# facebookresearch/metamorph

Hardware: AMD Instinct MI355X
Metric: train tokens/sec (LLaMA-3-8B + SigLIP-SO400M, seq2048, 256 img toks), whole job (higher is better)
Workload: dtype bf16

## Files before the change

### metamorph_amd/csrc/gemm_bf16.hip

```cpp
#include "gemm_common.h"
#include "splitk.h"
#include <type_traits>
#include <cstdlib>

namespace {

MM_DEV void gemm_epilogue_swiglu(f32x4 (&acc)[8][4], const GemmArgs& a, unsigned char* smem, int m0, int tn, int wm, int wn, int wave, int lane) {
    constexpr int TN = 64;
    const int fr = lane & 15, fq = lane >> 4;
    const int M = a.M, I = (int)a.res_mod;
    float* stg = (float*)smem + wave * (16 * TN);
    const int row_l = lane >> 2, k4 = lane & 3;
    uint16_t* gu = (uint16_t*)a.C;
    uint16_t* act = (uint16_t*)a.res;
    const int ch0 = tn * 128 + wn * 32;
#pragma unroll
    for (int i = 0; i < 8; ++i) {
        __builtin_amdgcn_fence(__ATOMIC_RELEASE, "wavefront");
        __builtin_amdgcn_wave_barrier();
#pragma unroll
        for (int j = 0; j < 4; ++j)
#pragma unroll
            for (int r = 0; r < 4; ++r) stg[(fq * 4 + r) * TN + j * 16 + fr] = acc[i][j][r];
        __builtin_amdgcn_fence(__ATOMIC_RELEASE, "wavefront");
        __builtin_amdgcn_wave_barrier();
        const int grow = m0 + wm * 128 + i * 16 + row_l;
        if (grow < M) {
            float g[8], u[8], o[8];
            const f32x4 g0 = *(const f32x4*)(stg + row_l * TN + k4 * 8), g1 = *(const f32x4*)(stg + row_l * TN + k4 * 8 + 4);
            const f32x4 u0 = *(const f32x4*)(stg + row_l * TN + 32 + k4 * 8), u1 = *(const f32x4*)(stg + row_l * TN + 32 + k4 * 8 + 4);
            g[0] = g0.x; g[1] = g0.y; g[2] = g0.z; g[3] = g0.w; g[4] = g1.x; g[5] = g1.y; g[6] = g1.z; g[7] = g1.w;
            u[0] = u0.x; u[1] = u0.y; u[2] = u0.z; u[3] = u0.w; u[4] = u1.x; u[5] = u1.y; u[6] = u1.z; u[7] = u1.w;
            const u32x4 gp = pack8(g), up = pack8(u);
            const int ch = ch0 + k4 * 8;
            *(u32x4*)(gu + (int64_t)grow * a.ldc + ch) = gp;
            *(u32x4*)(gu + (int64_t)grow * a.ldc + I + ch) = up;
            float gb[8], ub[8];
            unpack8(gp, gb);
            unpack8(up, ub);
#pragma unroll
            for (int e = 0; e < 8; ++e) o[e] = round_bf(gb[e] / (1.0f + __expf(-gb[e]))) * ub[e];
            *(u32x4*)(act + (int64_t)grow * a.ldr + ch) = pack8(o);
        }
    }
}

constexpr int SWB_TROW = 144;
constexpr int SWB_T = 3 * 32 * SWB_TROW;
constexpr int SWB_LDS = 32768 + 8 * SWB_T;
MM_DEV void gemm_epilogue_swiglu_bwd(f32x4 (&acc)[8][4], const GemmArgs& a, unsigned char* smem, int m0, int n0, int wm, int wn, int wave, int lane) {
    constexpr int TN = 64, PF = 4;
    typedef __attribute__((ext_vector_type(4))) short s16x4;
    typedef __attribute__((address_space(3))) s16x4* lds4_t;
    const int fr = lane & 15, fq = lane >> 4;
    const int M = a.M, I = a.N;
    float* stg = (float*)smem + wave * (16 * TN);
    unsigned char* tile = smem + 32768 + wave * SWB_T;
    const int row_l = lane >> 2, k4 = lane & 3;
    const uint16_t* gu = a.res;
    uint16_t* dgu = (uint16_t*)a.C;
    const int c_wave = n0 + wn * 64;
    if (c_wave >= I) return;
    const int row0 = m0 + wm * 128 + row_l;
    u32x4 gq[PF][2], uq[PF][2];
    auto fetch = [&](int i, int slot) {
        const int grow = row0 + i * 16;
#pragma unroll
        for (int j8 = 0; j8 < 2; ++j8) {
            const int64_t ro = (int64_t)min(grow, M - 1) * a.ldr + c_wave + k4 * 16 + j8 * 8;
            gq[slot][j8] = *(const u32x4*)(gu + ro);
            uq[slot][j8] = *(const u32x4*)(gu + ro + I);
        }
    };
#pragma unroll
    for (int i = 0; i < PF; ++i) fetch(i, i);
#pragma unroll
    for (int ib = 0; ib < 4; ++ib) {
#pragma unroll
        for (int half = 0; half < 2; ++half) {
            const int i = ib * 2 + half;
            __builtin_amdgcn_fence(__ATOMIC_RELEASE, "wavefront");
            __builtin_amdgcn_wave_barrier();
#pragma unroll
            for (int j = 0; j < 4; ++j)
#pragma unroll
                for (int r = 0; r < 4; ++r) stg[(fq * 4 + r) * TN + j * 16 + fr] = acc[i][j][r];
            __builtin_amdgcn_fence(__ATOMIC_RELEASE, "wavefront");
            __builtin_amdgcn_wave_barrier();
            const int grow = row0 + i * 16;
            const bool live = grow < M;
#pragma unroll
            for (int j8 = 0; j8 < 2; ++j8) {
                const int c = k4 * 16 + j8 * 8;
                float daf[8], g[8], u[8], dg[8], du[8], av[8], da[8];
                const f32x4 s0 = *(const f32x4*)(stg + row_l * TN + c), s1 = *(const f32x4*)(stg + row_l * TN + c + 4);
                daf[0] = s0.x; daf[1] = s0.y; daf[2] = s0.z; daf[3] = s0.w; daf[4] = s1.x; daf[5] = s1.y; daf[6] = s1.z; daf[7] = s1.w;
                unpack8(pack8(daf), da);
                unpack8(gq[i % PF][j8], g);
                unpack8(uq[i % PF][j8], u);
#pragma unroll
                for (int e = 0; e < 8; ++e) {
                    const float sg = 1.0f / (1.0f + __expf(-g[e]));
                    const float silu = g[e] * sg;
                    av[e] = round_bf(silu) * u[e];
                    du[e] = da[e] * round_bf(silu);
                    dg[e] = da[e] * u[e] * (sg * (1.0f + g[e] * (1.0f - sg)));
                }
                const u32x4 pg = pack8(dg), pu = pack8(du), pa = pack8(av);
                if (live) {
                    const int64_t wo = (int64_t)grow * a.ldc + c_wave + c;
                    *(u32x4*)(dgu + wo) = pg;
                    *(u32x4*)(dgu + wo + I) = pu;
                }
                unsigned char* tp = tile + (half * 16 + row_l) * SWB_TROW + c * 2;
                *(u32x4*)(tp) = pa;
                *(u32x4*)(tp + 32 * SWB_TROW) = pg;
                *(u32x4*)(tp + 64 * SWB_TROW) = pu;
            }
            if (i + PF < 8) fetch(i + PF, i % PF);
        }
        __builtin_amdgcn_fence(__ATOMIC_RELEASE, "wavefront");
        __builtin_amdgcn_wave_barrier();
        const int r_base = m0 + wm * 128 + ib * 32;
        const int s_l = fr >> 2, j_l = fr & 3;
        const unsigned char* tb = tile + (8 * (fr & 3) + (fr >> 2)) * SWB_TROW + fq * 8;
#pragma unroll
        for (int q = 0; q < 3; ++q) {
#pragma unroll
            for (int it = 0; it < 4; ++it) {
                const s16x4 lo = __builtin_amdgcn_ds_read_tr16_b64_v4i16((lds4_t)(tb + q * 32 * SWB_TROW + it * 32));
                const s16x4 hi = __builtin_amdgcn_ds_read_tr16_b64_v4i16((lds4_t)(tb + (q * 32 + 4) * SWB_TROW + it * 32));
                const int ch = c_wave + it * 16 + fq * 4 + j_l;
                const int r8 = r_base + 8 * s_l;
                if (r8 < M) {
                    typedef __attribute__((ext_vector_type(8))) short s16x8;
                    uint16_t* outp = (q == 0 ? a.aux0 : a.aux1) + (int64_t)(q == 2 ? I + ch : ch) * a.ld_aux;
                    *(s16x8*)(outp + r8) = s16x8{lo[0], lo[1], lo[2], lo[3], hi[0], hi[1], hi[2], hi[3]};
                }
            }
        }
    }
}

MM_DEV void gemm_epilogue_rope(f32x4 (&acc)[8][4], const GemmArgs& a, unsigned char* smem, int m0, int n0, int wm, int wn, int wave, int lane) {
    constexpr int TN = 64;
    const int fr = lane & 15, fq = lane >> 4;
    const int M = a.M, L = (int)a.ld_aux, n_rot = (int)a.res_mod;
    float* stg = (float*)smem + wave * (16 * TN);
    const int row_l = lane >> 2, k4 = lane & 3;
    uint16_t* out = (uint16_t*)a.C;
    const int32_t* pos_off = (const int32_t*)a.bias;
    const int d1 = (wn & 1) * 32 + k4 * 8;
    const int col1 = n0 + (wn >> 1) * 128 + d1;
    const bool rot = col1 < n_rot;
#pragma unroll
    for (int i = 0; i < 8; ++i) {
        __builtin_amdgcn_fence(__ATOMIC_RELEASE, "wavefront");
        __builtin_amdgcn_wave_barrier();
#pragma unroll
        for (int j = 0; j < 4; ++j)
#pragma unroll
            for (int r = 0; r < 4; ++r) stg[(fq * 4 + r) * TN + j * 16 + fr] = acc[i][j][r];
        __builtin_amdgcn_fence(__ATOMIC_RELEASE, "wavefront");
        __builtin_amdgcn_wave_barrier();
        const int grow = m0 + wm * 128 + i * 16 + row_l;
        if (grow < M) {
            float a1[8], a2[8], x1[8], x2[8];
            const f32x4 p0 = *(const f32x4*)(stg + row_l * TN + k4 * 8), p1 = *(const f32x4*)(stg + row_l * TN + k4 * 8 + 4);
            const f32x4 q0 = *(const f32x4*)(stg + row_l * TN + 32 + k4 * 8), q1 = *(const f32x4*)(stg + row_l * TN + 32 + k4 * 8 + 4);
            a1[0] = p0.x; a1[1] = p0.y; a1[2] = p0.z; a1[3] = p0.w; a1[4] = p1.x; a1[5] = p1.y; a1[6] = p1.z; a1[7] = p1.w;
            a2[0] = q0.x; a2[1] = q0.y; a2[2] = q0.z; a2[3] = q0.w; a2[4] = q1.x; a2[5] = q1.y; a2[6] = q1.z; a2[7] = q1.w;
            u32x4 w1 = pack8(a1), w2 = pack8(a2);
            if (rot) {
                unpack8(w1, x1);
                unpack8(w2, x2);
                const int b = grow / L;
                const int l = grow - b * L + (pos_off ? pos_off[b] : 0);
                float c[8], sn[8], y1[8], y2[8];
                unpack8(*(const u32x4*)(a.aux0 + (int64_t)l * 128 + d1), c);
                unpack8(*(const u32x4*)(a.aux1 + (int64_t)l * 128 + d1), sn);
#pragma unroll
                for (int e = 0; e < 8; ++e) {
                    y1[e] = round_bf(x1[e] * c[e]) + round_bf(-x2[e] * sn[e]);
                    y2[e] = round_bf(x2[e] * c[e]) + round_bf(x1[e] * sn[e]);
                }
                w1 = pack8(y1); w2 = pack8(y2);
            }
            *(u32x4*)(out + (int64_t)grow * a.ldc + col1) = w1;
            *(u32x4*)(out + (int64_t)grow * a.ldc + col1 + 64) = w2;
        }
    }
}

template <int BM, int BN, int WM, int WN, bool GLDS, int PIPE = 0>
__global__ __launch_bounds__(WM* WN * 64) void gemm_nt_kernel(GemmArgs a) {
    constexpr int NT = WM * WN * 64, NW = WM * WN;
    constexpr int TM = BM / WM, TN = BN / WN, FM = TM / 16, FN = TN / 16;
    constexpr int A_BYTES = BM * 128, B_BYTES = BN * 128, STAGE = A_BYTES + B_BYTES;
    constexpr int AV = BM * 8 / NT, BV = BN * 8 / NT;
    constexpr int AI = BM / 8 / NW, BI = BN / 8 / NW;
    constexpr int GM = 8;
    static_assert(FM >= 1 && FN >= 2 && (FN % 2) == 0, "tile shape");
    static_assert(AV >= 1 && BV >= 1 && AI >= 1 && BI >= 1, "thread/tile ratio");

    extern __shared__ __attribute__((aligned(16))) unsigned char smem[];

    const int total = a.ntm * a.ntn;
    const int bid = blockIdx.x;
    const int q8 = total >> 3, r8 = total & 7;
    const int xcd = bid & 7, idx = bid >> 3;
    const int logical = (xcd < r8 ? xcd * (q8 + 1) : r8 * (q8 + 1) + (xcd - r8) * q8) + idx;
    const int gsize = GM * a.ntn;
    const int grp = logical / gsize;
    const int first_m = grp * GM;
    const int gm = min(a.ntm - first_m, GM);
    const int in_g = logical - grp * gsize;
    const int tm = first_m + in_g % gm;
    const int tn = in_g / gm;
    const int m0 = tm * BM, n0 = tn * BN;

    const int tid = threadIdx.x, lane = tid & 63, wave = tid >> 6;
    const int wm = wave / WN, wn = wave % WN;
    const int fr = lane & 15, fq = lane >> 4;
    const int sl = a.kslice ? (int)blockIdx.y : 0;
    const uint16_t* Ab = a.A + (int64_t)sl * a.kslice;
    const uint16_t* Bb = a.B + (int64_t)sl * a.kslice;
    const int M = a.M, N = a.N, K = a.kslice ? min(a.kslice, a.K - sl * a.kslice) : a.K;
    const int nk = (K + 63) >> 6;

    f32x4 acc[FM][FN];
#pragma unroll
    for (int i = 0; i < FM; ++i)
#pragma unroll
        for (int j = 0; j < FN; ++j) acc[i][j] = f32x4{0.f, 0.f, 0.f, 0.f};

    const int sw0 = ((fq) ^ (fr & 7)) << 4;
    const int sw1 = ((4 + fq) ^ (fr & 7)) << 4;
    const int a_off = (wm * TM + fr) * 128;
    const int b_off = A_BYTES + (wn * TN + fr) * 128;

    u32x4 ra[AV], rb[BV];

    auto gload = [&](int kt) {
        const int k0 = kt << 6;
#pragma unroll
        for (int i = 0; i < AV; ++i) {
            const int v = tid + i * NT, row = v >> 3, c = v & 7;
            const int gr = min(m0 + row, M - 1), k = k0 + c * 8;
            ra[i] = (k < K) ? *(const u32x4*)(Ab + (int64_t)gr * a.lda + k) : u32x4{0u, 0u, 0u, 0u};
        }
#pragma unroll
        for (int i = 0; i < BV; ++i) {
            const int v = tid + i * NT, row = v >> 3, c = v & 7;
            const int gr = min(n0 + row, N - 1), k = k0 + c * 8;
            rb[i] = (k < K) ? *(const u32x4*)(Bb + (int64_t)gr * a.ldb + k) : u32x4{0u, 0u, 0u, 0u};
        }
    };
    auto lstore = [&](int buf) {
        unsigned char* sb = smem + buf * STAGE;
#pragma unroll
        for (int i = 0; i < AV; ++i) {
            const int v = tid + i * NT, row = v >> 3, c = v & 7;
            *(u32x4*)(sb + row * 128 + ((c ^ (row & 7)) << 4)) = ra[i];
        }
#pragma unroll
        for (int i = 0; i < BV; ++i) {
            const int v = tid + i * NT, row = v >> 3, c = v & 7;
            *(u32x4*)(sb + A_BYTES + row * 128 + ((c ^ (row & 7)) << 4)) = rb[i];
        }
    };
    const int wave_s = __builtin_amdgcn_readfirstlane(wave);
    const uint16_t* srcA[AI];
    const uint16_t* srcB[BI];
    {
        const int rin = lane >> 3;
        const int c = (lane & 7) ^ rin;
#pragma unroll
        for (int i = 0; i < AI; ++i)
            srcA[i] = Ab + (int64_t)min(m0 + (i * NW + wave_s) * 8 + rin, M - 1) * a.lda + c * 8;
#pragma unroll
        for (int i = 0; i < BI; ++i)
            srcB[i] = Bb + (int64_t)min(n0 + (i * NW + wave_s) * 8 + rin, N - 1) * a.ldb + c * 8;
    }
    auto gdma = [&](int kt, int buf) {
        const int64_t k0 = kt << 6;
        unsigned char* sb = smem + buf * STAGE + wave_s * 1024;
#pragma unroll
        for (int i = 0; i < AI; ++i)
            __builtin_amdgcn_global_load_lds((gptr_t)(srcA[i] + k0), (lptr_t)(sb + i * NW * 1024), 16, 0, 0);
#pragma unroll
        for (int i = 0; i < BI; ++i)
            __builtin_amdgcn_global_load_lds((gptr_t)(srcB[i] + k0), (lptr_t)(sb + A_BYTES + i * NW * 1024), 16, 0, 0);
    };

    if constexpr (PIPE == 0) {
    if constexpr (GLDS) {
        gdma(0, 0);
    } else {
        gload(0);
        lstore(0);
    }
    __syncthreads();
    int cur = 0;
    for (int kt = 0; kt < nk; ++kt) {
        const bool more = kt + 1 < nk;
        if (more) {
            if constexpr (GLDS) gdma(kt + 1, cur ^ 1);
            else gload(kt + 1);
        }
        const unsigned char* sb = smem + cur * STAGE;
#pragma unroll
        for (int kk = 0; kk < 2; ++kk) {
            const int sw = kk ? sw1 : sw0;
            bf16x8 af[FM], bf[FN];
#pragma unroll
            for (int i = 0; i < FM; ++i) af[i] = *(const bf16x8*)(sb + a_off + i * 2048 + sw);
#pragma unroll
            for (int j = 0; j < FN; ++j) bf[j] = *(const bf16x8*)(sb + b_off + j * 2048 + sw);
#pragma unroll
            for (int i = 0; i < FM; ++i)
#pragma unroll
                for (int j = 0; j < FN; ++j)
                    acc[i][j] = __builtin_amdgcn_mfma_f32_16x16x32_bf16(af[i], bf[j], acc[i][j], 0, 0, 0);
        }
        if constexpr (!GLDS) {
            if (more) lstore(cur ^ 1);
        }
        __syncthreads();
        cur ^= 1;
    }

    } else {
        static_assert(GLDS, "pipelined schedule uses LDS-DMA staging");
        static_assert(FM % 2 == 0, "pipelined schedule splits the A fragments in two halves");
        constexpr int HM = FM / 2;
        bf16x8 X[HM], Y[HM], P[FN], Q[FN];
        auto rdA = [&](bf16x8 (&af)[HM], int buf, int half, int kk) {
            const int sw = kk ? sw1 : sw0;
            const unsigned char* sb = smem + buf * STAGE + a_off + half * HM * 2048 + sw;
#pragma unroll
            for (int i = 0; i < HM; ++i) af[i] = *(const bf16x8*)(sb + i * 2048);
        };
        auto rdB = [&](bf16x8 (&bf)[FN], int buf, int kk) {
            const int sw = kk ? sw1 : sw0;
            const unsigned char* sb = smem + buf * STAGE + b_off + sw;
#pragma unroll
            for (int j = 0; j < FN; ++j) bf[j] = *(const bf16x8*)(sb + j * 2048);
        };
        auto mm = [&](const bf16x8 (&af)[HM], const bf16x8 (&bf)[FN], int half) {
            __builtin_amdgcn_s_setprio(1);
#pragma unroll
            for (int i = 0; i < HM; ++i)
#pragma unroll
                for (int j = 0; j < FN; ++j)
                    acc[half * HM + i][j] = __builtin_amdgcn_mfma_f32_16x16x32_bf16(af[i], bf[j], acc[half * HM + i][j], 0, 0, 0);
            __builtin_amdgcn_s_setprio(0);
        };
        gdma(0, 0);
        __syncthreads();
        if (nk > 1) gdma(1, 1);
        rdA(X, 0, 0, 0);
        rdB(P, 0, 0);
        int cur = 0;
        for (int kt = 0; kt < nk; ++kt) {
            rdA(Y, cur, 1, 0);
            __builtin_amdgcn_sched_barrier(0);
            mm(X, P, 0);
            __builtin_amdgcn_sched_barrier(0);
            rdA(X, cur, 0, 1);
            rdB(Q, cur, 1);
            __builtin_amdgcn_sched_barrier(0);
            mm(Y, P, 1);
            __builtin_amdgcn_sched_barrier(0);
            rdA(Y, cur, 1, 1);
            __builtin_amdgcn_sched_barrier(0);
            mm(X, Q, 0);
            __builtin_amdgcn_sched_barrier(0);
            __syncthreads();
            if (kt + 2 < nk) gdma(kt + 2, cur);
            if (kt + 1 < nk) {
                rdA(X, cur ^ 1, 0, 0);
                rdB(P, cur ^ 1, 0);
            }
            __builtin_amdgcn_sched_barrier(0);
            mm(Y, Q, 1);
            __builtin_amdgcn_sched_barrier(0);
            cur ^= 1;
        }
        __syncthreads();
    }

    if (a.kslice) {
        GemmArgs e = a;
        e.C = (float*)a.C + (int64_t)sl * a.M * a.ldc;
        gemm_epilogue<TM, TN, FM, FN>(acc, e, smem, m0, n0, wm, wn, wave, lane);
        return;
    }
    gemm_epilogue<TM, TN, FM, FN>(acc, a, smem, m0, n0, wm, wn, wave, lane);
}

template <int N> MM_DEV void wait_vmcnt() {
#if defined(MM355_SWB_ABL) && MM355_SWB_ABL == 3
    static_assert(N >= 0 && N <= 10, "unsupported count");
    asm volatile("s_waitcnt vmcnt(%0)" :: "n"(N) : "memory");
#else
    static_assert(N == 0 || N == 2 || N == 4 || N == 6 || N == 8, "unsupported count");
    if constexpr (N == 8) asm volatile("s_waitcnt vmcnt(8)" ::: "memory");
    else if constexpr (N == 6) asm volatile("s_waitcnt vmcnt(6)" ::: "memory");
    else if constexpr (N == 4) asm volatile("s_waitcnt vmcnt(4)" ::: "memory");
    else if constexpr (N == 2) asm volatile("s_waitcnt vmcnt(2)" ::: "memory");
    else asm volatile("s_waitcnt vmcnt(0)" ::: "memory");
#endif
}

template <int ABL = 0, bool SWI = false, bool SWB = false, bool ROPE = false>
MM_DEV void gemm_pp_tile(const GemmArgs& a, const int bid, unsigned char* smem) {
    constexpr int BM = 256, BN = 256, TM = 128, TN = 64, FM = 8, FN = 4;
    constexpr int BUF = (BM + BN) * 128;
    constexpr int A_BYTES = BM * 128;

    const int total = a.ntm * a.ntn;
    const int q8 = total >> 3, r8 = total & 7;
    const int xcd = bid & 7, idx = bid >> 3;
    const int logical = (xcd < r8 ? xcd * (q8 + 1) : r8 * (q8 + 1) + (xcd - r8) * q8) + idx;
    const int GM = a.gm;
    const int gsize = GM * a.ntn;
    const int grp = logical / gsize;
    const int first_m = grp * GM;
    const int gm = min(a.ntm - first_m, GM);
    const int in_g = logical - grp * gsize;
    const int tm = first_m + in_g % gm;
    const int tn = in_g / gm;
    const int m0 = tm * BM, n0 = tn * BN;

    const int tid = threadIdx.x, lane = tid & 63, wave = tid >> 6;
    const int wave_s = __builtin_amdgcn_readfirstlane(wave);
    const int wm = wave_s >> 2, wn = wave_s & 3;
    const int fr = lane & 15, fq = lane >> 4;
    const int M = a.M, N = a.N;
    const int nk = a.K >> 6;
#ifdef MM355_SWB_STAGGER
    if constexpr (SWB) {
        if (bid < 256) {
            const int ph = (bid >> 3) % MM355_SWB_PHASES;
            for (int i = 0; i < ph * MM355_SWB_STAGGER; ++i) __builtin_amdgcn_s_sleep(127);
        }
    }
#endif

    f32x4 acc[FM][FN];
#pragma unroll
    for (int i = 0; i < FM; ++i)
#pragma unroll
        for (int j = 0; j < FN; ++j) acc[i][j] = f32x4{0.f, 0.f, 0.f, 0.f};

    uint32_t src[4][2];
    int dst[4][2];
#pragma unroll
    for (int h = 0; h < 2; ++h) {
        const int q = wave_s + 8 * h;
#pragma unroll
        for (int kd = 0; kd < 4; ++kd) {
            const bool isA = kd == 0 || kd == 3;
            const int blk = isA ? (kd == 3) : (kd - 1);
            if (isA) {
                const int rin = lane >> 3, c = (lane & 7) ^ rin;
                const int row = h * 128 + blk * 64 + wave_s * 8;
                src[kd][h] = (uint32_t)((int64_t)(min(m0 + row + rin, M - 1) - m0) * a.lda * 2 + c * 16);
                dst[kd][h] = row * 128;
            } else {
                const int rin = lane >> 3, c = (lane & 7) ^ rin;
                const int row = (q >> 2) * 64 + blk * 32 + (q & 3) * 8;
                if constexpr (SWI) {
                    const int wrow = blk * (int)a.res_mod + tn * 128 + (q >> 2) * 32 + (q & 3) * 8 + rin;
                    src[kd][h] = (uint32_t)((int64_t)wrow * a.ldb * 2 + c * 16);
                } else if constexpr (ROPE) {
                    const int wrow = ((q >> 2) >> 1) * 128 + blk * 64 + ((q >> 2) & 1) * 32 + (q & 3) * 8 + rin;
                    src[kd][h] = (uint32_t)((int64_t)wrow * a.ldb * 2 + c * 16);
                } else {
                    src[kd][h] = (uint32_t)((int64_t)(min(n0 + row + rin, N - 1) - n0) * a.ldb * 2 + c * 16);
                }
                dst[kd][h] = A_BYTES + row * 128;
            }
        }
    }
    const uint16_t* baseA = a.A + (int64_t)m0 * a.lda;
    const uint16_t* baseB = SWI ? a.B : a.B + (int64_t)n0 * a.ldb;
    const __amdgpu_buffer_rsrc_t rsA = __builtin_amdgcn_make_buffer_rsrc((void*)baseA, 0, 0x7fffffff, 0x00020000);
    const __amdgpu_buffer_rsrc_t rsB = __builtin_amdgcn_make_buffer_rsrc((void*)baseB, 0, 0x7fffffff, 0x00020000);
    auto issue = [&](int kd, int tile) {
        unsigned char* sb = smem + (tile & 1) * BUF;
        const bool isA = kd == 0 || kd == 3;
#pragma unroll
        for (int h = 0; h < 2; ++h)
            __builtin_amdgcn_raw_ptr_buffer_load_lds(isA ? rsA : rsB, (lptr_t)(sb + dst[kd][h]), 16, src[kd][h],
                                                     (ABL == 3 ? (tile & 1) : tile) * 128, 0, 0);
    };

    const int sw0 = ((fq) ^ (fr & 7)) << 4;
    const int sw1 = ((4 + fq) ^ (fr & 7)) << 4;
    const int a_off = (wm * TM + fr) * 128;
    const int b_off = A_BYTES + (wn * TN + fr) * 128;
    bf16x8 A[2][4][2], B[2][2][2];
    auto rdA = [&](int ah, int tile) {
        const unsigned char* sb = smem + (tile & 1) * BUF + a_off + ah * 8192;
#pragma unroll
        for (int i = 0; i < 4; ++i) {
            A[ah][i][0] = *(const bf16x8*)(sb + i * 2048 + sw0);
            A[ah][i][1] = *(const bf16x8*)(sb + i * 2048 + sw1);
        }
    };
    auto rdB = [&](int bh, int tile) {
        const unsigned char* sb = smem + (tile & 1) * BUF + b_off + bh * 4096;
#pragma unroll
        for (int j = 0; j < 2; ++j) {
            B[bh][j][0] = *(const bf16x8*)(sb + j * 2048 + sw0);
            B[bh][j][1] = *(const bf16x8*)(sb + j * 2048 + sw1);
        }
    };
#if defined(MM355_SWB_ABL) && MM355_SWB_ABL == 3
    u32x4 swb_sink = u32x4{0u, 0u, 0u, 0u};
    auto swb_extra = [&](int pidx) -> int {
        int n = 0;
        const int row_l = lane >> 2, k4 = lane & 3;
        const int c_wave = n0 + wn * 64;
        if ((pidx & 7) == 0) {
            const int li = pidx >> 3, i = li >> 2, j8 = (li >> 1) & 1, gsel = li & 1;
            const int grow = min(m0 + wm * 128 + row_l + i * 16, M - 1);
            const uint16_t* pa = a.res + (int64_t)grow * a.ldr + min(c_wave, a.N - 64) + k4 * 16 + j8 * 8 + gsel * a.N;
            asm volatile("global_load_dwordx4 %0, %1, off" : "=v"(swb_sink) : "v"(pa) : "memory");
            ++n;
        }
        const int s_now = (pidx * 5) >> 4, s_prev = pidx ? ((pidx - 1) * 5) >> 4 : -1;
        if (s_now != s_prev) {
            const int si = s_now;
            uint16_t* pa;
            if (si < 32) {
                const int i = si >> 2, j8 = (si >> 1) & 1, gsel = si & 1;
                const int grow = min(m0 + wm * 128 + row_l + i * 16, M - 1);
                pa = (uint16_t*)a.C + (int64_t)grow * a.ldc + min(c_wave, a.N - 64) + k4 * 16 + j8 * 8 + gsel * a.N;
            } else {
                const int t = si - 32, q = t >> 4, it = (t >> 2) & 3, ib = t & 3;
                const int ch = min(c_wave, a.N - 64) + it * 16 + fq * 4 + (fr & 3);
                const int r8 = min(m0 + wm * 128 + ib * 32 + 8 * (fr >> 2), M - 8);
                pa = (q == 0 ? a.aux0 : a.aux1) + (int64_t)(q == 2 ? a.N + ch : ch) * a.ld_aux + r8;
            }
            asm volatile("global_store_dwordx4 %0, %1, off" :: "v"(pa), "v"(swb_sink) : "memory");
            ++n;
        }
        return n;
    };
#endif
    auto phase = [&](auto p_c, auto vm_c, auto issue_c, auto nexta_c, int tile, int st) {
        constexpr int P = decltype(p_c)::value, VM = decltype(vm_c)::value;
        constexpr bool ISSUE = decltype(issue_c)::value, NEXTA = decltype(nexta_c)::value;
        constexpr int ah = P >> 1, bh = (P == 1 || P == 2) ? 1 : 0;
        if constexpr (ABL != 2) {
            if constexpr (P == 0) rdB(0, tile);
            if constexpr (P == 1) rdB(1, tile);
            if constexpr (P == 2) rdA(1, tile);
            if constexpr (P == 3 && NEXTA) rdA(0, tile + 1);
        }
        if constexpr (ISSUE && ABL != 1) issue((P + 2) & 3, st);
#if defined(MM355_SWB_ABL) && MM355_SWB_ABL == 3
        if constexpr (SWB) {
            const int nx = swb_extra(tile * 4 + P);
            if (nx == 0) wait_vmcnt<VM>();
            else if (nx == 1) wait_vmcnt<VM + 1>();
            else wait_vmcnt<VM + 2>();
        } else
#endif
        if constexpr (ABL != 1) wait_vmcnt<VM>();
        __builtin_amdgcn_sched_barrier(0);
        __builtin_amdgcn_s_barrier();
        asm volatile("s_waitcnt lgkmcnt(0)" ::: "memory");
        __builtin_amdgcn_sched_barrier(0);
        __builtin_amdgcn_s_setprio(1);
#pragma unroll
        for (int kk = 0; kk < 2; ++kk)
#pragma unroll
            for (int i = 0; i < 4; ++i)
#pragma unroll
                for (int j = 0; j < 2; ++j)
                    acc[ah * 4 + i][bh * 2 + j] =
                        __builtin_amdgcn_mfma_f32_16x16x32_bf16(A[ah][i][kk], B[bh][j][kk], acc[ah * 4 + i][bh * 2 + j], 0, 0, 0);
        __builtin_amdgcn_s_setprio(0);
        __builtin_amdgcn_sched_barrier(0);
        __builtin_amdgcn_s_barrier();
    };
    using I0 = std::integral_constant<int, 0>; using I1 = std::integral_constant<int, 1>;
    using I2 = std::integral_constant<int, 2>; using I3 = std::integral_constant<int, 3>;
    using I4 = std::integral_constant<int, 4>; using I6 = std::integral_constant<int, 6>;
    using I8 = std::integral_constant<int, 8>;
    using T = std::true_type; using F = std::false_type;

#if defined(MM355_SWB_ABL) && MM355_SWB_ABL == 2
    if constexpr (SWB) {
        __syncthreads();
        gemm_epilogue_swiglu_bwd(acc, a, smem, m0, n0, wm, wn, wave, lane);
        return;
    }
#endif
#pragma unroll
    for (int kd = 0; kd < 4; ++kd) issue(kd, 0);
    issue(0, 1);
    issue(1, 1);
    wait_vmcnt<8>();
    __builtin_amdgcn_s_barrier();
    rdA(0, 0);
    if (wm == 1) __builtin_amdgcn_s_barrier();

    int t = 0;
    for (; t + 2 < nk; t += 2) {
        phase(I0{}, I8{}, T{}, T{}, t, t + 1);
        phase(I1{}, I8{}, T{}, T{}, t, t + 1);
        phase(I2{}, I8{}, T{}, T{}, t, t + 2);
        phase(I3{}, I8{}, T{}, T{}, t, t + 2);
        phase(I0{}, I8{}, T{}, T{}, t + 1, t + 2);
        phase(I1{}, I8{}, T{}, T{}, t + 1, t + 2);
        phase(I2{}, I8{}, T{}, T{}, t + 1, t + 3);
        phase(I3{}, I8{}, T{}, T{}, t + 1, t + 3);
    }
    phase(I0{}, I8{}, T{}, T{}, t, t + 1);
    phase(I1{}, I8{}, T{}, T{}, t, t + 1);
    phase(I2{}, I6{}, F{}, T{}, t, 0);
    phase(I3{}, I4{}, F{}, T{}, t, 0);
    phase(I0{}, I2{}, F{}, T{}, t + 1, 0);
    phase(I1{}, I0{}, F{}, T{}, t + 1, 0);
    phase(I2{}, I0{}, F{}, T{}, t + 1, 0);
    phase(I3{}, I0{}, F{}, F{}, t + 1, 0);
    if (wm == 0) __builtin_amdgcn_s_barrier();
    __syncthreads();
#if defined(MM355_SWB_ABL) && (MM355_SWB_ABL == 1 || MM355_SWB_ABL == 3)
    if constexpr (SWB) {
        float keep = 0.f;
#pragma unroll
        for (int i = 0; i < FM; ++i)
#pragma unroll
            for (int j = 0; j < FN; ++j) keep += acc[i][j][0] + acc[i][j][1] + acc[i][j][2] + acc[i][j][3];
        if (keep == 1.2345e-30f) ((float*)a.C)[tid] = keep;
        return;
    }
#endif
    if constexpr (SWI) gemm_epilogue_swiglu(acc, a, smem, m0, tn, wm, wn, wave, lane);
    else if constexpr (SWB) gemm_epilogue_swiglu_bwd(acc, a, smem, m0, n0, wm, wn, wave, lane);
    else if constexpr (ROPE) gemm_epilogue_rope(acc, a, smem, m0, n0, wm, wn, wave, lane);
    else gemm_epilogue<TM, TN, FM, FN>(acc, a, smem, m0, n0, wm, wn, wave, lane);
}

__global__ __launch_bounds__(512) void gemm_pp_swiglu_kernel(GemmArgs a) {
    extern __shared__ __attribute__((aligned(16))) unsigned char smem[];
    gemm_pp_tile<0, true>(a, blockIdx.x, smem);
}

__global__ __launch_bounds__(512) void gemm_pp_rope_kernel(GemmArgs a) {
    extern __shared__ __attribute__((aligned(16))) unsigned char smem[];
    gemm_pp_tile<0, false, false, true>(a, blockIdx.x, smem);
}

__global__ __launch_bounds__(512) void gemm_pp_swiglu_bwd_kernel(GemmArgs a) {
    extern __shared__ __attribute__((aligned(16))) unsigned char smem[];
    gemm_pp_tile<0, false, true>(a, blockIdx.x, smem);
}

template <int ABL = 0>
__global__ __launch_bounds__(512) void gemm_pp_kernel(GemmArgs a) {
    extern __shared__ __attribute__((aligned(16))) unsigned char smem[];
#ifdef MM355_PP_PERSIST
    const int total = a.ntm * a.ntn;
    for (int bid = blockIdx.x; bid < total; bid += gridDim.x) {
        gemm_pp_tile<ABL>(a, bid, smem);
        __syncthreads();
    }
#else
    gemm_pp_tile<ABL>(a, blockIdx.x, smem);
#endif
}

__global__ __launch_bounds__(512) void gemm_pp_pair_kernel(GemmArgs a0, GemmArgs a1, int n0) {
    extern __shared__ __attribute__((aligned(16))) unsigned char smem[];
    const int bid = blockIdx.x;
    if (bid < n0) gemm_pp_tile(a0, bid, smem);
    else gemm_pp_tile(a1, bid - n0, smem);
}

template <int BM, int BN, int WM, int WN, bool GLDS, int PIPE>
int launch_gemm(GemmArgs a, hipStream_t s);

constexpr int PP_LDS = 2 * (256 + 256) * 128;

int64_t pp_prepare(GemmArgs& a) {
    a.ntm = (a.M + 255) / 256;
    a.ntn = (a.N + 255) / 256;
    a.gm = 4;
    return (int64_t)a.ntm * a.ntn;
}

template <int ABL = 0>
int launch_gemm_pp_t(GemmArgs a, hipStream_t s) {
    static std::atomic<uint64_t> lds_ok{0};
    if (mm_ensure_dynamic_lds((const void*)gemm_pp_kernel<ABL>, PP_LDS, lds_ok) != MM355_OK) return MM355_ELAUNCH;
    const int64_t total = pp_prepare(a);
    if (total <= 0 || total > 0x7fffffff) return MM355_EINVAL;
#ifdef MM355_PP_PERSIST
    hipLaunchKernelGGL((gemm_pp_kernel<ABL>), dim3((unsigned)std::min<int64_t>(total, MM355_PP_PERSIST)), dim3(512), PP_LDS, s, a);
#else
    hipLaunchKernelGGL((gemm_pp_kernel<ABL>), dim3((unsigned)total), dim3(512), PP_LDS, s, a);
#endif
    return mm_launch_status();
}

int launch_gemm_pp_pair(GemmArgs a0, GemmArgs a1, hipStream_t s) {
    static std::atomic<uint64_t> lds_ok{0};
    if (mm_ensure_dynamic_lds((const void*)gemm_pp_pair_kernel, PP_LDS, lds_ok) != MM355_OK) return MM355_ELAUNCH;
    const int64_t n0 = pp_prepare(a0), n1 = pp_prepare(a1);
    if (n0 <= 0 || n1 <= 0 || n0 + n1 > 0x7fffffff) return MM355_EINVAL;
    hipLaunchKernelGGL(gemm_pp_pair_kernel, dim3((unsigned)(n0 + n1)), dim3(512), PP_LDS, s, a0, a1, (int)n0);
    return mm_launch_status();
}

bool pp_eligible(const GemmArgs& a) {
    if (a.K < 128 || (a.K & 127)) return false;
    const int64_t ea = (256 * a.lda + a.K) * 2;
    const int64_t eb = (256 * a.ldb + a.K) * 2;
    return ea < 0x7fffffffLL && eb < 0x7fffffffLL;
}

int launch_gemm_pp(GemmArgs a, hipStream_t s) {
    if (!pp_eligible(a)) return launch_gemm<256, 256, 2, 4, true, 1>(a, s);
    return launch_gemm_pp_t(a, s);
}

template <int BM, int BN, int WM, int WN, bool GLDS, int PIPE = 0>
int launch_gemm(GemmArgs a, hipStream_t s) {
    constexpr int STAGE = (BM + BN) * 128;
    constexpr int LDS = 2 * STAGE;
    auto kern = gemm_nt_kernel<BM, BN, WM, WN, GLDS, PIPE>;
    static std::atomic<uint64_t> lds_ok{0};
    if (mm_ensure_dynamic_lds((const void*)kern, LDS, lds_ok) != MM355_OK) return MM355_ELAUNCH;
    a.ntm = (a.M + BM - 1) / BM;
    a.ntn = (a.N + BN - 1) / BN;
    const int64_t total = (int64_t)a.ntm * a.ntn;
    if (total <= 0 || total > 0x7fffffff) return MM355_EINVAL;
    hipLaunchKernelGGL(kern, dim3((unsigned)total), dim3(WM * WN * 64), LDS, s, a);
    return mm_launch_status();
}

__global__ __launch_bounds__(256) void transpose_kernel(const uint16_t* __restrict__ in, int64_t ld_in, int rows, int cols,
                                                        uint16_t* __restrict__ out, int64_t ld_out) {
    __shared__ uint16_t tile[64][64 + 2];
    const int r0 = blockIdx.y * 64, c0 = blockIdx.x * 64;
    const int tid = threadIdx.x;
#pragma unroll
    for (int i = 0; i < 2; ++i) {
        const int v = tid + i * 256, r = v >> 3, c = (v & 7) * 8;
        const int gr = r0 + r, gc = c0 + c;
        uint16_t tmp[8];
        if (gr < rows && gc + 8 <= cols) {
            *(u32x4*)tmp = *(const u32x4*)(in + (int64_t)gr * ld_in + gc);
        } else {
#pragma unroll
            for (int e = 0; e < 8; ++e) tmp[e] = (gr < rows && gc + e < cols) ? in[(int64_t)gr * ld_in + gc + e] : (uint16_t)0;
        }
#pragma unroll
        for (int e = 0; e < 8; ++e) tile[r][c + e] = tmp[e];
    }
    __syncthreads();
#pragma unroll
    for (int i = 0; i < 2; ++i) {
        const int v = tid + i * 256, c = v >> 3, r = (v & 7) * 8;
        const int gc = c0 + c, gr = r0 + r;
        if (gc >= cols) continue;
        uint16_t tmp[8];
#pragma unroll
        for (int e = 0; e < 8; ++e) tmp[e] = tile[r + e][c];
        if (gr + 8 <= rows && ((ld_out & 7) == 0)) {
            *(u32x4*)(out + (int64_t)gc * ld_out + gr) = *(const u32x4*)tmp;
        } else {
            for (int e = 0; e < 8; ++e)
                if (gr + e < rows) out[(int64_t)gc * ld_out + gr + e] = tmp[e];
        }
    }
}

__global__ __launch_bounds__(256) void colsum_kernel(const uint16_t* __restrict__ x, int64_t ld, int M, int N, float* __restrict__ out) {
    __shared__ float part[4][64];
    const int cq = threadIdx.x & 63, rp = threadIdx.x >> 6;
    const int c = blockIdx.x * 64 + cq;
    float s = 0.f;
    if (c < N)
        for (int r = rp; r < M; r += 4) s += bf2f(x[(int64_t)r * ld + c]);
    part[rp][cq] = s;
    __syncthreads();
    if (rp == 0 && c < N) out[c] += (part[0][cq] + part[1][cq]) + (part[2][cq] + part[3][cq]);
}

__global__ __launch_bounds__(1024) void colsum8_kernel(const uint16_t* __restrict__ x, int64_t ld, int M, int N, float* __restrict__ out) {
    __shared__ float part[128][65];
    const int cg = threadIdx.x & 7, rp = threadIdx.x >> 3;
    const int c0 = blockIdx.x * 64 + cg * 8;
    float s[8] = {0.f, 0.f, 0.f, 0.f, 0.f, 0.f, 0.f, 0.f};
    if (c0 < N)
        for (int r = rp; r < M; r += 128) {
            float f[8];
            unpack8(*(const u32x4*)(x + (int64_t)r * ld + c0), f);
#pragma unroll
            for (int e = 0; e < 8; ++e) s[e] += f[e];
        }
#pragma unroll
    for (int e = 0; e < 8; ++e) part[rp][cg * 8 + e] = s[e];
    __syncthreads();
    const int c = blockIdx.x * 64 + threadIdx.x;
    if (threadIdx.x < 64 && c < N) {
        float t = 0.f;
        for (int p = 0; p < 128; ++p) t += part[p][threadIdx.x];
        out[c] += t;
    }
}

}

namespace {
__global__ __launch_bounds__(256) void splitk_reduce_kernel(const float* __restrict__ part, int S, int M, int N, const uint16_t* __restrict__ res,
                                                            int64_t ldr, uint16_t* __restrict__ out, int64_t ldc) {
    const int nv = N >> 3;
    const int64_t total = (int64_t)M * nv, plane = (int64_t)M * N;
    for (int64_t i = blockIdx.x * 256ll + threadIdx.x; i < total; i += (int64_t)gridDim.x * 256) {
        const int m = (int)(i / nv), c = (int)(i % nv) * 8;
        float v[8];
        const float* p = part + (int64_t)m * N + c;
        const f32x4 a0 = *(const f32x4*)p, a1 = *(const f32x4*)(p + 4);
        v[0] = a0.x; v[1] = a0.y; v[2] = a0.z; v[3] = a0.w; v[4] = a1.x; v[5] = a1.y; v[6] = a1.z; v[7] = a1.w;
        for (int s = 1; s < S; ++s) {
            const f32x4 b0 = *(const f32x4*)(p + s * plane), b1 = *(const f32x4*)(p + s * plane + 4);
            v[0] += b0.x; v[1] += b0.y; v[2] += b0.z; v[3] += b0.w; v[4] += b1.x; v[5] += b1.y; v[6] += b1.z; v[7] += b1.w;
        }
// ... 470 lines not shown
```

### metamorph_amd/csrc/gemm_common.h

```cpp
#pragma once
#include "mm355_common.h"

namespace {

struct GemmArgs {
    const uint16_t* A;
    const uint16_t* B;
    void* C;
    const uint16_t* bias;
    const uint16_t* res;
    int64_t lda, ldb, ldc, ldr, res_mod;
    int M, N, K;
    uint32_t flags;
    int ntm, ntn;
    int gm;
    uint16_t* aux0;
    uint16_t* aux1;
    int64_t ld_aux;
    int kslice;
};

MM_DEV void gemm_tile_map(const int ntm, const int ntn, const int GM, const int bid, int& tm, int& tn) {
    const int total = ntm * ntn;
    const int q8 = total >> 3, r8 = total & 7;
    const int xcd = bid & 7, idx = bid >> 3;
    const int logical = (xcd < r8 ? xcd * (q8 + 1) : r8 * (q8 + 1) + (xcd - r8) * q8) + idx;
    const int gsize = GM * ntn;
    const int grp = logical / gsize;
    const int first_m = grp * GM;
    const int gm = min(ntm - first_m, GM);
    const int in_g = logical - grp * gsize;
    tm = first_m + in_g % gm;
    tn = in_g / gm;
}

__device__ __attribute__((noinline)) void epi_scalar(void* C, int64_t ldc, const uint16_t* bias, const uint16_t* res, int64_t ldr,
                                                     uint32_t fl, int N, int grow, int c, int64_t rr, float v0, float v1,
                                                     float v2, float v3, float v4, float v5, float v6, float v7) {
    const float v[8] = {v0, v1, v2, v3, v4, v5, v6, v7};
    for (int e = 0; e < 8; ++e) {
        const int ce = c + e;
        if (ce >= N) break;
        float x = v[e];
        if (fl & MM355_GEMM_BIAS) x += bf2f(bias[ce]);
        if (fl & MM355_GEMM_GELU_ERF) x = gelu_erf_f(x);
        else if (fl & MM355_GEMM_GELU_TANH) x = gelu_tanh_f(x);
        if (fl & MM355_GEMM_RESIDUAL) x += bf2f(res[rr * ldr + ce]);
        if (fl & MM355_GEMM_OUT_F32) {
            float* p = (float*)C + (int64_t)grow * ldc + ce;
            if (fl & MM355_GEMM_ACCUMULATE) x += *p;
            *p = x;
        } else {
            uint16_t* p = (uint16_t*)C + (int64_t)grow * ldc + ce;
            if (fl & MM355_GEMM_ACCUMULATE) x += bf2f(*p);
            *p = f2bf(x);
        }
    }
}

typedef const __attribute__((address_space(1))) void* gptr_t;
typedef __attribute__((address_space(3))) void* lptr_t;

MM_DEV void epi_store8(const GemmArgs& a, const uint32_t fl, const bool vec_ok, const int grow, const int64_t rr, const int c, float (&v)[8]) {
    const int N = a.N;
    uint16_t* Cb = (uint16_t*)a.C;
    float* Cf = (float*)a.C;
    const bool full = (c + 8 <= N) && vec_ok;
    if (full) {
        if (fl & MM355_GEMM_BIAS) {
            float b[8];
            unpack8(*(const u32x4*)(a.bias + c), b);
#pragma unroll
            for (int e = 0; e < 8; ++e) v[e] += b[e];
        }
        if (fl & MM355_GEMM_GELU_ERF) {
#pragma unroll
            for (int e = 0; e < 8; ++e) v[e] = gelu_erf_f(v[e]);
        } else if (fl & MM355_GEMM_GELU_TANH) {
#pragma unroll
            for (int e = 0; e < 8; ++e) v[e] = gelu_tanh_f(v[e]);
        }
        if (fl & MM355_GEMM_RESIDUAL) {
            float b[8];
            unpack8(*(const u32x4*)(a.res + rr * a.ldr + c), b);
#pragma unroll
            for (int e = 0; e < 8; ++e) v[e] += b[e];
        }
        if (fl & MM355_GEMM_OUT_F32) {
            float* p = Cf + (int64_t)grow * a.ldc + c;
            if (fl & MM355_GEMM_ACCUMULATE) {
                const f32x4 o0 = *(const f32x4*)p, o1 = *(const f32x4*)(p + 4);
                v[0] += o0.x; v[1] += o0.y; v[2] += o0.z; v[3] += o0.w;
                v[4] += o1.x; v[5] += o1.y; v[6] += o1.z; v[7] += o1.w;
            }
            *(f32x4*)p = f32x4{v[0], v[1], v[2], v[3]};
            *(f32x4*)(p + 4) = f32x4{v[4], v[5], v[6], v[7]};
        } else {
            uint16_t* p = Cb + (int64_t)grow * a.ldc + c;
            if (fl & MM355_GEMM_ACCUMULATE) {
                float b[8];
                unpack8(*(const u32x4*)p, b);
#pragma unroll
                for (int e = 0; e < 8; ++e) v[e] += b[e];
            }
            *(u32x4*)p = pack8(v);
        }
    } else {
        epi_scalar(a.C, a.ldc, a.bias, a.res, a.ldr, fl, N, grow, c, rr, v[0], v[1], v[2], v[3], v[4], v[5], v[6], v[7]);
    }
}

template <int TM, int TN, int FM, int FN>
MM_DEV void gemm_epilogue(f32x4 (&acc)[FM][FN], const GemmArgs& a, unsigned char* smem, int m0, int n0, int wm, int wn, int wave, int lane) {
    const int fr = lane & 15, fq = lane >> 4;
    const int M = a.M, N = a.N;
    constexpr int CPL = TN / 4;
    float* stg = (float*)smem + wave * (16 * TN);
    const uint32_t fl = a.flags;
    const int row_l = lane >> 2, col_l = (lane & 3) * CPL;
    uint16_t* Cb = (uint16_t*)a.C;
    float* Cf = (float*)a.C;
    const bool vec_ok = ((a.ldc & 7) == 0) && (!(fl & MM355_GEMM_RESIDUAL) || (a.ldr & 7) == 0);
#pragma unroll
    for (int i = 0; i < FM; ++i) {
        __builtin_amdgcn_fence(__ATOMIC_RELEASE, "wavefront");
        __builtin_amdgcn_wave_barrier();
#pragma unroll
        for (int j = 0; j < FN; ++j)
#pragma unroll
            for (int r = 0; r < 4; ++r) stg[(fq * 4 + r) * TN + j * 16 + fr] = acc[i][j][r];
        __builtin_amdgcn_fence(__ATOMIC_RELEASE, "wavefront");
        __builtin_amdgcn_wave_barrier();
        const int grow = m0 + wm * TM + i * 16 + row_l;
        if (grow < M) {
            const int64_t rr = (fl & MM355_GEMM_RESIDUAL) ? (a.res_mod > 0 ? (int64_t)(grow % a.res_mod) : (int64_t)grow) : 0;
#pragma unroll
            for (int j = 0; j < CPL / 8; ++j) {
                const int c = n0 + wn * TN + col_l + j * 8;
                if (c >= N) continue;
                float v[8];
                const f32x4 s0 = *(const f32x4*)(stg + row_l * TN + col_l + j * 8);
                const f32x4 s1 = *(const f32x4*)(stg + row_l * TN + col_l + j * 8 + 4);
                v[0] = s0.x; v[1] = s0.y; v[2] = s0.z; v[3] = s0.w;
                v[4] = s1.x; v[5] = s1.y; v[6] = s1.z; v[7] = s1.w;
                epi_store8(a, fl, vec_ok, grow, rr, c, v);
            }
        }
    }
}

}
```

Measured before the change: 26650.

## Specialize interior GEMM and RoPE epilogues with prefetched residual/accumulate and cos/sin loads

Adds template-specialized epilogues for full interior tiles, chosen by a runtime switch over the flag combination. Residual, accumulator and bias operands are prefetched into registers several row-fragments ahead, and per-element bounds and flag checks are dropped. The RoPE epilogue gets an interior path that loads all cos/sin rows up front. The cost is more register pressure, a larger binary from many instantiations, and possible occupancy loss.

New measurement: 26690 (median of 4 runs). Within noise of the previous version (+0.1%).

```diff
diff --git a/metamorph_amd/csrc/gemm_bf16.hip b/metamorph_amd/csrc/gemm_bf16.hip
--- a/metamorph_amd/csrc/gemm_bf16.hip
+++ b/metamorph_amd/csrc/gemm_bf16.hip
@@ -142,6 +142,59 @@
     }
 }
 
+template <bool POS>
+MM_DEV void gemm_epilogue_rope_interior(f32x4 (&acc)[8][4], const GemmArgs& a, unsigned char* smem, int m0, int wm, int wave, int lane, int d1, int col1) {
+    constexpr int TN = 64;
+    const int fr = lane & 15, fq = lane >> 4;
+    const int L = (int)a.ld_aux;
+    float* stg = (float*)smem + wave * (16 * TN);
+    const int row_l = lane >> 2, k4 = lane & 3;
+    uint16_t* out = (uint16_t*)a.C;
+    const int32_t* pos_off = (const int32_t*)a.bias;
+    const int row0 = m0 + wm * 128 + row_l;
+    int l[8];
+#pragma unroll
+    for (int i = 0; i < 8; ++i) {
+        const int b = (row0 + i * 16) / L;
+        l[i] = row0 + i * 16 - b * L;
+        if constexpr (POS) l[i] += pos_off[b];
+    }
+    u32x4 cq[8], sq[8];
+#pragma unroll
+    for (int i = 0; i < 8; ++i) {
+        cq[i] = *(const u32x4*)(a.aux0 + (int64_t)l[i] * 128 + d1);
+        sq[i] = *(const u32x4*)(a.aux1 + (int64_t)l[i] * 128 + d1);
+    }
+#pragma unroll
+    for (int i = 0; i < 8; ++i) {
+        __builtin_amdgcn_fence(__ATOMIC_RELEASE, "wavefront");
+        __builtin_amdgcn_wave_barrier();
+#pragma unroll
+        for (int j = 0; j < 4; ++j)
+#pragma unroll
+            for (int r = 0; r < 4; ++r) stg[(fq * 4 + r) * TN + j * 16 + fr] = acc[i][j][r];
+        __builtin_amdgcn_fence(__ATOMIC_RELEASE, "wavefront");
+        __builtin_amdgcn_wave_barrier();
+        const int grow = row0 + i * 16;
+        float a1[8], a2[8], x1[8], x2[8], c[8], sn[8], y1[8], y2[8];
+        const f32x4 p0 = *(const f32x4*)(stg + row_l * TN + k4 * 8), p1 = *(const f32x4*)(stg + row_l * TN + k4 * 8 + 4);
+        const f32x4 q0 = *(const f32x4*)(stg + row_l * TN + 32 + k4 * 8), q1 = *(const f32x4*)(stg + row_l * TN + 32 + k4 * 8 + 4);
+        a1[0] = p0.x; a1[1] = p0.y; a1[2] = p0.z; a1[3] = p0.w; a1[4] = p1.x; a1[5] = p1.y; a1[6] = p1.z; a1[7] = p1.w;
+        a2[0] = q0.x; a2[1] = q0.y; a2[2] = q0.z; a2[3] = q0.w; a2[4] = q1.x; a2[5] = q1.y; a2[6] = q1.z; a2[7] = q1.w;
+        unpack8(pack8(a1), x1);
+        unpack8(pack8(a2), x2);
+        unpack8(cq[i], c);
+        unpack8(sq[i], sn);
+#pragma unroll
+        for (int e = 0; e < 8; ++e) {
+            y1[e] = round_bf(x1[e] * c[e]) + round_bf(-x2[e] * sn[e]);
+            y2[e] = round_bf(x2[e] * c[e]) + round_bf(x1[e] * sn[e]);
+        }
+        *(u32x4*)(out + (int64_t)grow * a.ldc + col1) = pack8(y1);
+        *(u32x4*)(out + (int64_t)grow * a.ldc + col1 + 64) = pack8(y2);
+    }
+}
+
 MM_DEV void gemm_epilogue_rope(f32x4 (&acc)[8][4], const GemmArgs& a, unsigned char* smem, int m0, int n0, int wm, int wn, int wave, int lane) {
     constexpr int TN = 64;
     const int fr = lane & 15, fq = lane >> 4;
@@ -153,6 +206,11 @@
     const int d1 = (wn & 1) * 32 + k4 * 8;
     const int col1 = n0 + (wn >> 1) * 128 + d1;
     const bool rot = col1 < n_rot;
+    if (m0 + 256 <= M && n0 + (wn >> 1) * 128 < n_rot) {
+        if (pos_off) gemm_epilogue_rope_interior<true>(acc, a, smem, m0, wm, wave, lane, d1, col1);
+        else gemm_epilogue_rope_interior<false>(acc, a, smem, m0, wm, wave, lane, d1, col1);
+        return;
+    }
 #pragma unroll
     for (int i = 0; i < 8; ++i) {
         __builtin_amdgcn_fence(__ATOMIC_RELEASE, "wavefront");
@@ -413,7 +471,7 @@
 #endif
 }
 
-template <int ABL = 0, bool SWI = false, bool SWB = false, bool ROPE = false>
+template <int ABL = 0, bool SWI = false, bool SWB = false, bool ROPE = false, bool PAIR = false>
 MM_DEV void gemm_pp_tile(const GemmArgs& a, const int bid, unsigned char* smem) {
     constexpr int BM = 256, BN = 256, TM = 128, TN = 64, FM = 8, FN = 4;
     constexpr int BUF = (BM + BN) * 128;
@@ -645,7 +703,25 @@
     if constexpr (SWI) gemm_epilogue_swiglu(acc, a, smem, m0, tn, wm, wn, wave, lane);
     else if constexpr (SWB) gemm_epilogue_swiglu_bwd(acc, a, smem, m0, n0, wm, wn, wave, lane);
     else if constexpr (ROPE) gemm_epilogue_rope(acc, a, smem, m0, n0, wm, wn, wave, lane);
-    else gemm_epilogue<TM, TN, FM, FN>(acc, a, smem, m0, n0, wm, wn, wave, lane);
+    else if constexpr (PAIR) gemm_epilogue<TM, TN, FM, FN>(acc, a, smem, m0, n0, wm, wn, wave, lane);
+    else {
+        const uint32_t fl = a.flags;
+        const bool interior = m0 + BM <= M && n0 + BN <= N && (a.ldc & 7) == 0 && (!(fl & MM355_GEMM_RESIDUAL) || (a.ldr & 7) == 0);
+        const int set = interior ? ((fl & MM355_GEMM_BIAS) ? 1 : 0) | ((fl & MM355_GEMM_RESIDUAL) ? 2 : 0) | ((fl & MM355_GEMM_ACCUMULATE) ? 4 : 0) |
+                                       ((fl & MM355_GEMM_OUT_F32) ? 8 : 0) | ((fl & (MM355_GEMM_GELU_ERF | MM355_GEMM_GELU_TANH)) ? 16 : 0) : 0;
+#define MM355_EPI_SET(S)                                                                                                               \
+    case S:                                                                                                                            \
+        gemm_epilogue_interior<TM, TN, FM, FN, ((S) & 1) != 0, ((S) & 16) != 0, ((S) & 2) != 0, ((S) & 4) != 0, ((S) & 8) != 0>(       \
+            acc, a, smem, m0, n0, wm, wn, wave, lane);                                                                                 \
+        break;
+        switch (set) {
+            MM355_EPI_SET(1) MM355_EPI_SET(2) MM355_EPI_SET(3) MM355_EPI_SET(4) MM355_EPI_SET(5) MM355_EPI_SET(6) MM355_EPI_SET(7)
+            MM355_EPI_SET(9) MM355_EPI_SET(10) MM355_EPI_SET(11) MM355_EPI_SET(12) MM355_EPI_SET(13) MM355_EPI_SET(14) MM355_EPI_SET(15)
+            MM355_EPI_SET(17) MM355_EPI_SET(19) MM355_EPI_SET(25) MM355_EPI_SET(27)
+            default: gemm_epilogue<TM, TN, FM, FN>(acc, a, smem, m0, n0, wm, wn, wave, lane);
+        }
+#undef MM355_EPI_SET
+    }
 }
 
 __global__ __launch_bounds__(512) void gemm_pp_swiglu_kernel(GemmArgs a) {
@@ -680,8 +756,8 @@
 __global__ __launch_bounds__(512) void gemm_pp_pair_kernel(GemmArgs a0, GemmArgs a1, int n0) {
     extern __shared__ __attribute__((aligned(16))) unsigned char smem[];
     const int bid = blockIdx.x;
-    if (bid < n0) gemm_pp_tile(a0, bid, smem);
-    else gemm_pp_tile(a1, bid - n0, smem);
+    if (bid < n0) gemm_pp_tile<0, false, false, false, true>(a0, bid, smem);
+    else gemm_pp_tile<0, false, false, false, true>(a1, bid - n0, smem);
 }
 
 template <int BM, int BN, int WM, int WN, bool GLDS, int PIPE>
diff --git a/metamorph_amd/csrc/gemm_common.h b/metamorph_amd/csrc/gemm_common.h
--- a/metamorph_amd/csrc/gemm_common.h
+++ b/metamorph_amd/csrc/gemm_common.h
@@ -149,4 +149,101 @@
     }
 }
 
-}
+template <int TM, int TN, int FM, int FN, bool BIAS, bool GELU, bool RES, bool ACC, bool F32>
+MM_DEV void gemm_epilogue_interior(f32x4 (&acc)[FM][FN], const GemmArgs& a, unsigned char* smem, int m0, int n0, int wm, int wn, int wave, int lane) {
+    const int fr = lane & 15, fq = lane >> 4;
+    constexpr int CPL = TN / 4, NJ = CPL / 8;
+    constexpr int RB = NJ * ((RES ? 4 : 0) + (ACC ? (F32 ? 8 : 4) : 0));
+    constexpr int BUDGET = GELU ? 32 : 64;
+    constexpr int PF = RB == 0 ? 0 : (BUDGET / RB < FM ? BUDGET / RB : FM);
+    constexpr int NS = PF ? PF : 1;
+    float* stg = (float*)smem + wave * (16 * TN);
+    const uint32_t fl = a.flags;
+    const int row_l = lane >> 2, col_l = (lane & 3) * CPL;
+    const int row0 = m0 + wm * TM + row_l, col0 = n0 + wn * TN + col_l;
+    const uint32_t rmod = (RES && a.res_mod > 0 && a.res_mod < 0x80000000LL) ? (uint32_t)a.res_mod : 0x80000000u;
+    u32x4 bq[NJ], rq[NS][NJ], cq[NS][NJ];
+    f32x4 cf[NS][NJ][2];
+    if constexpr (BIAS) {
+#pragma unroll
+        for (int j = 0; j < NJ; ++j) bq[j] = *(const u32x4*)(a.bias + col0 + j * 8);
+    }
+    auto fetch = [&](int i, int slot) {
+        const int grow = row0 + i * 16;
+#pragma unroll
+        for (int j = 0; j < NJ; ++j) {
+            if constexpr (RES) {
+                const int64_t rr = (int64_t)((uint32_t)grow % rmod);
+                rq[slot][j] = *(const u32x4*)(a.res + rr * a.ldr + col0 + j * 8);
+            }
+            if constexpr (ACC && F32) {
+                const float* p = (const float*)a.C + (int64_t)grow * a.ldc + col0 + j * 8;
+                cf[slot][j][0] = *(const f32x4*)p;
+                cf[slot][j][1] = *(const f32x4*)(p + 4);
+            }
+            if constexpr (ACC && !F32) cq[slot][j] = *(const u32x4*)((const uint16_t*)a.C + (int64_t)grow * a.ldc + col0 + j * 8);
+        }
+    };
+#pragma unroll
+    for (int i = 0; i < PF; ++i) fetch(i, i);
+#pragma unroll
+    for (int i = 0; i < FM; ++i) {
+        __builtin_amdgcn_fence(__ATOMIC_RELEASE, "wavefront");
+        __builtin_amdgcn_wave_barrier();
+#pragma unroll
+        for (int j = 0; j < FN; ++j)
+#pragma unroll
+            for (int r = 0; r < 4; ++r) stg[(fq * 4 + r) * TN + j * 16 + fr] = acc[i][j][r];
+        __builtin_amdgcn_fence(__ATOMIC_RELEASE, "wavefront");
+        __builtin_amdgcn_wave_barrier();
+        const int grow = row0 + i * 16;
+        const int slot = i % NS;
+#pragma unroll
+        for (int j = 0; j < NJ; ++j) {
+            float v[8], b[8];
+            const f32x4 s0 = *(const f32x4*)(stg + row_l * TN + col_l + j * 8);
+            const f32x4 s1 = *(const f32x4*)(stg + row_l * TN + col_l + j * 8 + 4);
+            v[0] = s0.x; v[1] = s0.y; v[2] = s0.z; v[3] = s0.w;
+            v[4] = s1.x; v[5] = s1.y; v[6] = s1.z; v[7] = s1.w;
+            if constexpr (BIAS) {
+                unpack8(bq[j], b);
+#pragma unroll
+                for (int e = 0; e < 8; ++e) v[e] += b[e];
+            }
+            if constexpr (GELU) {
+                if (fl & MM355_GEMM_GELU_ERF) {
+#pragma unroll
+                    for (int e = 0; e < 8; ++e) v[e] = gelu_erf_f(v[e]);
+                } else {
+#pragma unroll
+                    for (int e = 0; e < 8; ++e) v[e] = gelu_tanh_f(v[e]);
+                }
+            }
+            if constexpr (RES) {
+                unpack8(rq[slot][j], b);
+#pragma unroll
+                for (int e = 0; e < 8; ++e) v[e] += b[e];
+            }
+            if constexpr (F32) {
+                float* p = (float*)a.C + (int64_t)grow * a.ldc + col0 + j * 8;
+                if constexpr (ACC) {
+                    const f32x4 o0 = cf[slot][j][0], o1 = cf[slot][j][1];
+                    v[0] += o0.x; v[1] += o0.y; v[2] += o0.z; v[3] += o0.w;
+                    v[4] += o1.x; v[5] += o1.y; v[6] += o1.z; v[7] += o1.w;
+                }
+                *(f32x4*)p = f32x4{v[0], v[1], v[2], v[3]};
+                *(f32x4*)(p + 4) = f32x4{v[4], v[5], v[6], v[7]};
+            } else {
+                if constexpr (ACC) {
+                    unpack8(cq[slot][j], b);
+#pragma unroll
+                    for (int e = 0; e < 8; ++e) v[e] += b[e];
+                }
+                *(u32x4*)((uint16_t*)a.C + (int64_t)grow * a.ldc + col0 + j * 8) = pack8(v);
+            }
+        }
+        if (PF && i + PF < FM) fetch(i + PF, slot);
+    }
+}
+
+}
```
